# WHOIGit/ifcb_classifier

Measured on AMD Instinct MI355X. Metric: train images/sec, inception_v3 299^2 IFCB ROIs, higher is better.
Workload: dtype bf16; 1 GPU; inception_v3 100-class bf16 TRAIN, batch 256 per GPU, synthetic u8 ROIs h,w~U{32..299} resized on-GPU to 299x299 (BASELINE.json configs[1]); global_batch=256, parallelism=dp1, program_lanes=4, IFCBK_LANES=4, weight_gradient_lanes=1, optimizer=adam lr=1e-3, loss=CE + 0.4*CE_aux, input_pipeline=preprocess then step on one stream

## Files before the change

### ifcb_classifier_amd/csrc/conv_common.h

```cpp
#pragma once
#include "common.h"

namespace {

struct ConvArgs {
    const void* x;
    const void* w;
    void* y;
    float* part;
    const float* ep_scale;
    const float* ep_shift;
    const void* ep_res;
    int ep_ldr, ep_relu;
    const void* bs_raw;
    const float *bs_mean, *bs_invstd, *bs_scale, *bs_shift;
    int bs_ld;
    const void* pad_;
    unsigned xbytes, wbytes;
    int H, W, C, ldx;
    int K, R, S;
    int P, Q, ldy;
    int ostr_h, ostr_w, base_h, base_w, ish, isw;
    int M, Kg;
    int accumulate;
    int seg_n, seg_end[4], seg_ld[4], seg_aff[4];
    void* seg_y[4];
    int PQ;
    int tilesN;
    int wKg, wSfull, w_rbase, w_sbase;
    int oH, oW, o_a, o_b;
    fastdiv_t fPQ, fQ;
    int tr;
    fastdiv_t fP;
    int dbg;
};

typedef const __attribute__((address_space(1))) void* gptr_t;
typedef __attribute__((address_space(3))) void* lptr_t;

template <class T> struct Mma;
template <> struct Mma<bf16_t> {
    typedef bf16x8_t frag_t;
    __device__ static __forceinline__ void run(const frag_t& a, const frag_t& b, f32x4_t& c) {
        c = __builtin_amdgcn_mfma_f32_16x16x32_bf16(a, b, c, 0, 0, 0);
    }
    __device__ static __forceinline__ void pack4(bf16_t* p, const f32x4_t& v) {
        uint2 u;
        u.x = pack2bf(v[0], v[1]);
        u.y = pack2bf(v[2], v[3]);
        *reinterpret_cast<uint2*>(p) = u;
    }
};
template <> struct Mma<float> {
    typedef f32x4_t frag_t;
    __device__ static __forceinline__ void run(const frag_t& a, const frag_t& b, f32x4_t& c) {
#pragma unroll
        for (int j = 0; j < 4; ++j) c = __builtin_amdgcn_mfma_f32_16x16x4f32(a[j], b[j], c, 0, 0, 0);
    }
    __device__ static __forceinline__ void pack4(float* p, const f32x4_t& v) { *reinterpret_cast<f32x4_t*>(p) = v; }
};

__device__ __forceinline__ void lds_dma16(__amdgpu_buffer_rsrc_t rs, lptr_t dst, unsigned voff, int soff) {
    __builtin_amdgcn_raw_ptr_buffer_load_lds(rs, dst, 16, voff, soff, 0, 0);
}

template <int N>
__device__ __forceinline__ void wait_vmcnt() {
    asm volatile("s_waitcnt vmcnt(%0)" ::"n"(N) : "memory");
}


template <class T, int BM, int BN, int NTHREADS, int MODE>
__device__ __forceinline__ void conv_epilogue_store(const ConvArgs& a, T* sC, float* sRed, const int t, const int lane, const int wave,
                                                    const int m0, const int n0, const int mtile) {
    constexpr bool BSTAT = MODE == 3;
    constexpr int ES = (int)sizeof(T);
    constexpr int CE = 16 / ES;
    constexpr int NW = NTHREADS / 64;
    constexpr int CPR = BN / CE;
    constexpr int CPRP = CPR <= 4 ? 4 : CPR <= 8 ? 8 : CPR <= 16 ? 16 : 32;
    constexpr int LDC = BN + CE;
    {
        constexpr int RPP = NTHREADS / CPRP;
        const int cc = t & (CPRP - 1);
        const int r0 = t / CPRP;
        const bool cvalid = (cc < CPR) && (n0 + cc * CE < a.K);
        typedef float f32x2_t __attribute__((ext_vector_type(2)));
        f32x2_t s1p[CE / 2], s2p[CE / 2];
#pragma unroll
        for (int j = 0; j < CE / 2; ++j) s1p[j] = s2p[j] = f32x2_t{0.f, 0.f};
        if (cvalid) {
            const int nn = n0 + cc * CE;
            float bmu[CE], bis[CE], bsc[CE], bsh[CE];
            if (BSTAT) {
#pragma unroll
                for (int j = 0; j < CE; ++j) {
                    bmu[j] = a.bs_mean[nn + j];
                    bis[j] = a.bs_invstd[nn + j];
                    bsc[j] = a.bs_scale[nn + j];
                    bsh[j] = a.bs_shift[nn + j];
                }
            }
            float sc[CE], sh[CE];
            if (a.ep_scale) {
#pragma unroll
                for (int j = 0; j < CE; ++j) {
                    sc[j] = a.ep_scale[nn + j];
                    sh[j] = a.ep_shift[nn + j];
                }
            }
            T* segbase = (T*)a.y + nn;
            int segld = a.ldy;
            bool seg_aff = true;
            if (MODE == 4) {
                int si = 0;
#pragma unroll
                for (int q = 0; q < 3; ++q)
                    if (q + 1 < a.seg_n && nn >= a.seg_end[q]) si = q + 1;
                segbase = (T*)a.seg_y[si] + (nn - (si ? a.seg_end[si - 1] : 0));
// ... 128 lines not shown
```

### ifcb_classifier_amd/csrc/conv_igemm.hip

```cpp
#include "conv_common.h"
#include <stdlib.h>

namespace {

template <class T, int NT, int WM, int NSTAGE, int MODE>
__global__ __launch_bounds__(128 * WM) void conv_igemm(ConvArgs a) {
    constexpr bool STRIDED = MODE == 1;
    constexpr int ES = (int)sizeof(T);
    constexpr int CE = 16 / ES;
    constexpr int BK = 128 / ES;
    typedef typename Mma<T>::frag_t frag_t;
    constexpr int NW = 2 * WM;
    constexpr int NTHREADS = 64 * NW;
    constexpr int BM = 64 * WM;
    constexpr int BN = 32 * NT;
    constexpr int JB = (NT * 4 + NW - 1) / NW;
    constexpr int G = 4 + JB;
    constexpr int D = NSTAGE - 1;
    constexpr int LDC = BN + CE;
    constexpr int STAGE = (BM + BN) * BK;
    constexpr int STAGE_BYTES = NSTAGE * STAGE * ES;
    constexpr int CT_BYTES = BM * LDC * ES + NW * BN * 2 * 4;
    constexpr int MAIN_BYTES = STAGE_BYTES > CT_BYTES ? STAGE_BYTES : CT_BYTES;
    constexpr int DUMMY_BYTES = (JB * NW > NT * 4) ? 1024 : 0;
    __shared__ __attribute__((aligned(16))) unsigned char smem[MAIN_BYTES + DUMMY_BYTES];
    T* sStage = reinterpret_cast<T*>(smem);
    T* sC = reinterpret_cast<T*>(smem);
    float* sRed = reinterpret_cast<float*>(smem + BM * LDC * ES);
    T* sDummy = reinterpret_cast<T*>(smem + MAIN_BYTES);

    const int t = threadIdx.x;
    const int lane = t & 63;
    const int wave = __builtin_amdgcn_readfirstlane(t >> 6);
    const int wm = wave >> 1, wn = wave & 1;
    const int bid = (int)xcd_remap(blockIdx.x, gridDim.x);
    const int mtile = bid / a.tilesN, ntile = bid - mtile * a.tilesN;
    const int m0 = mtile * BM, n0 = ntile * BN;

    const __amdgpu_buffer_rsrc_t rsA = __builtin_amdgcn_make_buffer_rsrc((void*)a.x, 0, a.xbytes, 0x00020000);
    const __amdgpu_buffer_rsrc_t rsB = __builtin_amdgcn_make_buffer_rsrc((void*)a.w, 0, a.wbytes, 0x00020000);
    constexpr unsigned OOB = 0x80000000u;
    const int lrow8 = lane >> 3;
    const int csrc = (lane & 7) ^ lrow8;
    int off0[4], bh[4], bw[4];
#pragma unroll
    for (int j = 0; j < 4; ++j) {
        int m = m0 + (wave * 4 + j) * 8 + lrow8;
        bool rv = m < a.M;
        int mm = rv ? m : 0;
        int n = (int)fdiv((uint32_t)mm, a.fPQ);
        int rem = mm - n * a.PQ;
        int p = (int)fdiv((uint32_t)rem, a.fQ);
        int q = rem - p * a.Q;
        bh[j] = rv ? p * a.ostr_h + a.base_h : -(1 << 24);
        bw[j] = q * a.ostr_w + a.base_w;
        off0[j] = STRIDED ? n * a.H * a.W * a.ldx : ((n * a.H + bh[j]) * a.W + bw[j]) * a.ldx;
    }
    int kc, kr, ks, tapoff;
    {
        kc = csrc * CE;
        kr = 0;
        ks = 0;
        while (kc >= a.C) {
            kc -= a.C;
            if (++ks == a.S) { ks = 0; ++kr; }
        }
        tapoff = (kr * a.W + ks) * a.ldx + kc;
    }
    int wk = MODE == 2 ? ((a.w_rbase + 2 * kr) * a.wSfull + a.w_sbase + 2 * ks) * a.C + kc : 0;
    unsigned woff[JB];
    bool gvalid[JB];
#pragma unroll
    for (int j = 0; j < JB; ++j) {
        int grp = j * NW + wave;
        gvalid[j] = grp < NT * 4;
        int n = n0 + grp * 8 + lrow8;
        woff[j] = (gvalid[j] && n < a.K) ? (MODE == 2 ? (unsigned)(n * a.wKg) : (unsigned)(n * a.Kg + csrc * CE)) * (unsigned)ES : OOB;
    }
    const int nk = (a.Kg + BK - 1) / BK;
    const int hmask = (1 << a.ish) - 1, wmask = (1 << a.isw) - 1;
    const int rowstep = a.W * a.ldx, colwrap = a.S * a.ldx;
    const int wrowskip = MODE == 2 ? (2 * a.wSfull - 2 * a.S) * a.C : 0;

    const bool plain = (MODE == 0 || MODE == 3 || MODE == 4) && a.R == 1 && a.S == 1 && a.base_h == 0 && a.base_w == 0;
    unsigned va[4];
#pragma unroll
    for (int j = 0; j < 4; ++j) va[j] = bh[j] >= 0 ? (unsigned)(off0[j] + csrc * CE) * (unsigned)ES : OOB;
    const bool ktail_ok = (nk - 1) * BK + csrc * CE < a.Kg;

#define ISSUE_TILE(kt, stage)                                                                              \
    {                                                                                                      \
        T* dstA = sStage + (stage) * STAGE;                                                                \
        T* dstB = dstA + BM * BK;                                                                          \
        if (plain) {                                                                                       \
            const bool cut = (kt) == nk - 1 && !ktail_ok;                                                  \
            _Pragma("unroll") for (int j = 0; j < 4; ++j)                                                  \
                lds_dma16(rsA, (lptr_t)(dstA + (wave * 4 + j) * 8 * BK), cut ? OOB : va[j], (kt) * 128);   \
        } else {                                                                                           \
            const bool kvalid = kr < a.R;                                                                  \
            _Pragma("unroll") for (int j = 0; j < 4; ++j) {                                                \
                int hr = bh[j] + kr, wr = bw[j] + ks;                                                      \
                unsigned voff;                                                                             \
                if (STRIDED) {                                                                             \
                    bool v = kvalid && hr >= 0 && wr >= 0 && ((hr & hmask) == 0) && ((wr & wmask) == 0);   \
                    int hi = hr >> a.ish, wi = wr >> a.isw;                                                \
                    v = v && hi < a.H && wi < a.W;                                                         \
                    voff = v ? (unsigned)(off0[j] + (hi * a.W + wi) * a.ldx + kc) * (unsigned)ES : OOB;    \
                } else {                                                                                   \
                    bool v = kvalid && (unsigned)hr < (unsigned)a.H && (unsigned)wr < (unsigned)a.W;       \
                    voff = v ? (unsigned)(off0[j] + tapoff) * (unsigned)ES : OOB;                          \
                }                                                                                          \
                __builtin_amdgcn_raw_ptr_buffer_load_lds(rsA, (lptr_t)(dstA + (wave * 4 + j) * 8 * BK), 16, voff, 0, 0, 0); \
            }                                                                                              \
        }                                                                                                  \
        if (MODE == 2) {                                                                                   \
            const bool kv2 = ((kt) * BK + csrc * CE) < a.Kg;                                               \
            _Pragma("unroll") for (int j = 0; j < JB; ++j) {                                               \
                unsigned voff = (kv2 && woff[j] != OOB) ? woff[j] + (unsigned)wk * (unsigned)ES : OOB;     \
// ... 246 lines not shown
                    sh[j] = nv ? a.ep_shift[ncol + nt * 16 + j] : 0.f;
                }
            }
            f32x2_t s1[2] = {f32x2_t{0.f, 0.f}, f32x2_t{0.f, 0.f}}, s2[2] = {f32x2_t{0.f, 0.f}, f32x2_t{0.f, 0.f}};
#pragma unroll
            for (int mt = 0; mt < 4; ++mt) {
                f32x4_t v = acc[nt][mt];
                if (a.ep_scale) {
#pragma unroll
                    for (int j = 0; j < 4; ++j) {
                        v[j] = bf2f(f2bf(v[j])) * sc[j] + sh[j];
                        if (a.ep_relu) v[j] = fmaxf(v[j], 0.f);
                    }
                }
                uint2 u;
                u.x = pack2bf(v[0], v[1]);
                u.y = pack2bf(v[2], v[3]);
                if (mv[mt] && nv) *reinterpret_cast<uint2*>(row[mt] + nt * 16) = u;
                const f32x2_t lo = {__uint_as_float(u.x << 16), __uint_as_float(u.x & 0xffff0000u)};
                const f32x2_t hi = {__uint_as_float(u.y << 16), __uint_as_float(u.y & 0xffff0000u)};
                s1[0] += lo; s1[1] += hi;
                s2[0] += lo * lo; s2[1] += hi * hi;
            }
            if (a.part) {
#pragma unroll
                for (int off = 1; off < 16; off <<= 1)
#pragma unroll
                    for (int h = 0; h < 2; ++h)
#pragma unroll
                        for (int j = 0; j < 2; ++j) {
                            s1[h][j] += __shfl_xor(s1[h][j], off);
                            s2[h][j] += __shfl_xor(s2[h][j], off);
                        }
                if (frow == 0 && nv) {
                    float* prow = a.part + ((size_t)(mtile * 2 + wm) * 2) * a.K + ncol + nt * 16;
#pragma unroll
                    for (int j = 0; j < 4; ++j) {
                        prow[j] = s1[j >> 1][j & 1];
                        prow[a.K + j] = s2[j >> 1][j & 1];
                    }
                }
            }
        }
    }
}

int pick_nt(int K, int maxnt) {
    static int force = -1;
    if (force < 0) { const char* e = getenv("IFCBK_CONV_NT"); force = e ? atoi(e) : 0; }
    if (force > 0 && force <= maxnt) return force;
    int best = 1;
    long bestc = -1;
    for (int nt = 1; nt <= maxnt; ++nt) {
        int bn = 32 * nt;
        long c = (long)cdiv(K, bn) * (bn + 48);
        if (bestc < 0 || c < bestc || (c == bestc && nt > best)) { bestc = c; best = nt; }
    }
    return best;
}

int check_desc(ifcbk_ctx* ctx, const ifcbk_conv_desc* d, bool dgrad = false) {
    if (!d) IFCBK_FAIL(ctx, IFCBK_EINVAL, "conv: null desc");
    if (d->dtype != IFCBK_BF16 && d->dtype != IFCBK_F32) IFCBK_FAIL(ctx, IFCBK_EUNSUPPORTED, "conv: dtype must be bf16 or f32");
    const int ce = dtype_chunk(d->dtype), es = dtype_esize(d->dtype);
    if (d->C % ce || d->K % ce || d->ldx % ce || d->ldy % ce || d->C <= 0 || d->K <= 0)
        IFCBK_FAIL(ctx, IFCBK_EINVAL, "conv: C=%d K=%d ldx=%d ldy=%d must be positive multiples of %d", d->C, d->K, d->ldx, d->ldy, ce);
    if (d->stride_h < 1 || d->stride_w < 1 || (dgrad && (d->stride_h > 2 || d->stride_w > 2)))
        IFCBK_FAIL(ctx, IFCBK_EINVAL, "conv: stride must be >= 1 (1 or 2 for the input gradient)");
    int P = (d->H + 2 * d->pad_h - d->R) / d->stride_h + 1, Q = (d->W + 2 * d->pad_w - d->S) / d->stride_w + 1;
    if (P != d->P || Q != d->Q) IFCBK_FAIL(ctx, IFCBK_EINVAL, "conv: P,Q=%d,%d inconsistent (expect %d,%d)", d->P, d->Q, P, Q);
    if ((int64_t)d->N * d->P * d->Q * d->ldy * es >= (1ll << 31) || (int64_t)d->N * d->H * d->W * d->ldx * es >= (1ll << 31))
        IFCBK_FAIL(ctx, IFCBK_EINVAL, "conv: a tensor exceeds the 2 GiB buffer-descriptor window");
    return 0;
}

int pick_wm(int M, int K) {
    static int force = -1;
    if (force < 0) { const char* e = getenv("IFCBK_CONV_WM"); force = e ? atoi(e) : 0; }
    (void)M; (void)K;
    return force == 4 ? 4 : 2;
}

template <class T, int NT, int WM, int NSTAGE>
void launch(const ConvArgs& a, hipStream_t st) {
    int tilesM = cdiv(a.M, 64 * WM);
    dim3 grid((unsigned)(tilesM * a.tilesN)), block(128 * WM);
    if (a.seg_n) hipLaunchKernelGGL((conv_igemm<T, NT, WM, NSTAGE, 4>), grid, block, 0, st, a);
    else if (a.bs_raw) hipLaunchKernelGGL((conv_igemm<T, NT, WM, NSTAGE, 3>), grid, block, 0, st, a);
    else if (a.wKg) hipLaunchKernelGGL((conv_igemm<T, NT, WM, NSTAGE, 2>), grid, block, 0, st, a);
    else if (a.ish | a.isw) hipLaunchKernelGGL((conv_igemm<T, NT, WM, NSTAGE, 1>), grid, block, 0, st, a);
    else hipLaunchKernelGGL((conv_igemm<T, NT, WM, NSTAGE, 0>), grid, block, 0, st, a);
}

int ws_min_steps() {
    static int v = -1;
    if (v < 0) { const char* e = getenv("IFCBK_CONV_WS"); v = e ? atoi(e) : 4; }
    return v;
}
int num_cus();
int ws_max_tiles() {
    static int v = -1;
    if (v < 0) { const char* e = getenv("IFCBK_CONV_WS_TILES"); v = e ? atoi(e) : 2 * num_cus(); }
    return v;
}
bool ws_shape_ok(int dtype, int M, int K, int Kg) {
    const int ms = ws_min_steps();
    if (ms <= 0 || dtype != IFCBK_BF16 || pick_wm(M, K) != 2 || cdiv(Kg, 64) < ms) return false;
    const int nt = pick_nt(K, 6);
    return (int64_t)cdiv(M, 128) * cdiv(K, 32 * nt) <= ws_max_tiles();
}
int num_cus() {
    static int n = 0;
    if (!n) {
        int dev = 0;
        hipDeviceProp_t pr;
        if (hipGetDevice(&dev) == hipSuccess && hipGetDeviceProperties(&pr, dev) == hipSuccess) n = pr.multiProcessorCount;
        if (n <= 0) n = 256;
    }
    return n;
}

template <int NT>
void launch_ws(const ConvArgs& a, hipStream_t st) {
    const int total = cdiv(a.M, 128) * a.tilesN;
    const int grid = total < num_cus() ? total : num_cus();
    hipLaunchKernelGGL((conv_ws<NT>), dim3((unsigned)grid), dim3(512), 0, st, a, total);
}

bool big_ok(const ConvArgs& a) { return !a.wKg && !(a.ish | a.isw); }
bool pp3_ok(const ConvArgs& a) {
    return big_ok(a) && !a.seg_n && !a.bs_raw && !a.accumulate && !a.ep_res && (a.ep_scale == nullptr || a.part == nullptr);
}

int run(ifcbk_ctx* ctx, ConvArgs& a, int dtype, hipStream_t st) {
    const bool f32 = dtype == IFCBK_F32;
    if (!a.wKg && !(a.ish | a.isw) && a.ostr_h == 1 && a.ostr_w == 1 && !a.seg_n && !a.accumulate && !a.ep_res && a.PQ > 0) {
        const int N = a.M / a.PQ;
        if (ifcbk_conv_flat_rows(dtype, N, a.H, a.W, a.C, a.K, a.R, a.S, -a.base_h, -a.base_w, a.P, a.Q) > 0)
            return ifcbk_conv_flat_launch(ctx, &a, N, st);
    }
    if (big_ok(a) && a.ostr_h == 1 && a.ostr_w == 1 && !a.seg_n && a.PQ > 0) {
        const int N = a.M / a.PQ;
        if (ifcbk_conv_slab_plan(dtype, N, a.H, a.W, a.C, a.K, a.R, a.S, -a.base_h, -a.base_w, a.P, a.Q) > 0)
            return ifcbk_conv_slab_launch(ctx, &a, N, st);
    }
    if (pp3_ok(a) && ifcbk_conv_pp3_plan(dtype, a.M, a.K, a.Kg, a.ep_scale ? 1 : 0)) return ifcbk_conv_pp3_launch(ctx, &a, st);
    {
        int bmt = 0, btn = 0;
        if (big_ok(a) && ifcbk_conv_big_plan(dtype, a.M, a.K, a.Kg, &bmt, &btn)) return ifcbk_conv_big_launch(ctx, &a, bmt, btn, st);
    }
    int wm = f32 ? 2 : pick_wm(a.M, a.K);
    int nt = pick_nt(a.K, f32 ? 4 : (wm == 4 ? 5 : 6));
    a.tilesN = cdiv(a.K, 32 * nt);
    if ((int64_t)cdiv(a.M, 64 * wm) * a.tilesN >= (1ll << 31)) IFCBK_FAIL(ctx, IFCBK_EINVAL, "conv: grid too large");
    if (ws_shape_ok(dtype, a.M, a.K, a.Kg) && !a.seg_n && !a.bs_raw && !a.wKg && !(a.ish | a.isw) && !a.accumulate && !a.ep_res) {
        switch (nt) {
            case 1: launch_ws<1>(a, st); break;
            case 2: launch_ws<2>(a, st); break;
            case 3: launch_ws<3>(a, st); break;
            case 4: launch_ws<4>(a, st); break;
            case 5: launch_ws<5>(a, st); break;
            default: launch_ws<6>(a, st); break;
        }
        IFCBK_LAUNCH_CHECK(ctx, "conv_ws");
        return 0;
    }
    if (f32) {
        switch (nt) {
            case 1: launch<float, 1, 2, 2>(a, st); break;
            case 2: launch<float, 2, 2, 2>(a, st); break;
            case 3: launch<float, 3, 2, 2>(a, st); break;
            default: launch<float, 4, 2, 2>(a, st); break;
        }
    } else if (wm == 4) {
        switch (nt) {
            case 1: launch<bf16_t, 1, 4, 3>(a, st); break;
            case 2: launch<bf16_t, 2, 4, 3>(a, st); break;
            case 3: launch<bf16_t, 3, 4, 3>(a, st); break;
            case 4: launch<bf16_t, 4, 4, 3>(a, st); break;
            default: launch<bf16_t, 5, 4, 3>(a, st); break;
        }
    } else {
        switch (nt) {
            case 1: launch<bf16_t, 1, 2, 2>(a, st); break;
            case 2: launch<bf16_t, 2, 2, 2>(a, st); break;
            case 3: launch<bf16_t, 3, 2, 2>(a, st); break;
            case 4: launch<bf16_t, 4, 2, 2>(a, st); break;
            case 5: launch<bf16_t, 5, 2, 2>(a, st); break;
            default: launch<bf16_t, 6, 2, 2>(a, st); break;
        }
    }
    IFCBK_LAUNCH_CHECK(ctx, "conv_igemm");
    return 0;
}

}

int ifcbk_num_cus() { return num_cus(); }

int ifcbk_conv_fwd_nt(int K, int M) { return pick_nt(K, pick_wm(M, K) == 4 ? 5 : 6); }

int ifcbk_conv_f32_nt(int K) { return pick_nt(K, 4); }

int ifcbk_conv_fwd_wm(int M, int K) { return pick_wm(M, K); }

bool ifcbk_conv_ws_shape(int dtype, int M, int K, int Kg) { return ws_shape_ok(dtype, M, K, Kg); }

static bool fwd_rows(const ifcbk_conv_desc* d) {
    return ifcbk_conv_rows_ok(d->dtype, d->C, d->K, d->R, d->S, d->stride_h, d->stride_w, d->pad_h, d->pad_w, d->Q);
}

extern "C" int ifcbk_conv2d_fwd_mblocks(const ifcbk_conv_desc* d) {
    if (fwd_rows(d)) return ifcbk_conv_rows_blocks(d->N, d->P);
    int M = d->N * d->P * d->Q;
    if (d->stride_h == 1 && d->stride_w == 1)
        if (int fs = ifcbk_conv_flat_rows(d->dtype, d->N, d->H, d->W, d->C, d->K, d->R, d->S, d->pad_h, d->pad_w, d->P, d->Q)) return fs;
    if (d->stride_h == 1 && d->stride_w == 1)
        if (int smt = ifcbk_conv_slab_plan(d->dtype, d->N, d->H, d->W, d->C, d->K, d->R, d->S, d->pad_h, d->pad_w, d->P, d->Q)) return cdiv(M, 32 * smt);
    if (ifcbk_conv_pp3_plan(d->dtype, M, d->K, d->R * d->S * d->C, 0)) return 2 * cdiv(M, 256);
    {
        int bmt = 0, btn = 0;
        if (ifcbk_conv_big_plan(d->dtype, M, d->K, d->R * d->S * d->C, &bmt, &btn)) return cdiv(M, 32 * bmt);
    }
    if (ws_shape_ok(d->dtype, M, d->K, d->R * d->S * d->C)) return 2 * cdiv(M, 128);
    return cdiv(M, 64 * pick_wm(M, d->K));
}

struct FwdSegs { int n, end[4], ld[4], aff[4]; void* y[4]; };
static int conv_fwd_impl(ifcbk_ctx* ctx, const ifcbk_conv_desc* d, const void* x, const void* w, void* y, float* bn_part,
                         const float* scale, const float* shift, const void* residual, int ldr, int relu, void* stream,
                         const FwdSegs* seg = nullptr);

extern "C" int ifcbk_conv2d_fwd_affine_segments(ifcbk_ctx* ctx, const ifcbk_conv_desc* d, const void* x, const void* w, int nseg,
                                                void* const* ys, const int32_t* ldys, const int32_t* ksegs, const int32_t* affine,
                                                const float* scale, const float* shift, void* stream) {
    if (!d || nseg < 1 || nseg > 4 || !ys || !ldys || !ksegs || !affine || !scale || !shift)
        IFCBK_FAIL(ctx, IFCBK_EINVAL, "conv2d_fwd_affine_segments: bad args");
    FwdSegs sg;
    sg.n = nseg;
    int end = 0;
    const int ce = dtype_chunk(d->dtype);
    for (int q = 0; q < 4; ++q) {
        const bool live = q < nseg;
        if (live) {
            if (!ys[q] || ksegs[q] <= 0 || ksegs[q] % ce || ldys[q] % ce)
                IFCBK_FAIL(ctx, IFCBK_EINVAL, "conv2d_fwd_affine_segments: segment %d: null / size not a multiple of %d", q, ce);
            end += ksegs[q];
        }
        sg.end[q] = end; sg.ld[q] = live ? ldys[q] : 0; sg.aff[q] = live ? affine[q] : 0; sg.y[q] = live ? ys[q] : nullptr;
    }
    if (end != d->K) IFCBK_FAIL(ctx, IFCBK_EINVAL, "conv2d_fwd_affine_segments: segment sizes sum to %d, K=%d", end, d->K);
    return conv_fwd_impl(ctx, d, x, w, ys[0], nullptr, scale, shift, nullptr, 0, 1, stream, &sg);
}

extern "C" int ifcbk_conv2d_fwd(ifcbk_ctx* ctx, const ifcbk_conv_desc* d, const void* x, const void* w, void* y,
                                float* bn_part, void* stream) {
    return conv_fwd_impl(ctx, d, x, w, y, bn_part, nullptr, nullptr, nullptr, 0, 0, stream);
}

extern "C" int ifcbk_conv2d_fwd_affine(ifcbk_ctx* ctx, const ifcbk_conv_desc* d, const void* x, const void* w, void* y,
                                       const float* scale, const float* shift, const void* residual, int ldr, int relu,
                                       void* stream) {
    if (!scale || !shift) IFCBK_FAIL(ctx, IFCBK_EINVAL, "conv2d_fwd_affine: scale/shift required");
    return conv_fwd_impl(ctx, d, x, w, y, nullptr, scale, shift, residual, ldr, relu, stream);
}

extern "C" int ifcbk_conv2d_fwd_affine_maxpool_ok(const ifcbk_conv_desc* d) {
    return d && ifcbk_conv_rows_pool_ok(d->dtype, d->C, d->K, d->R, d->S, d->stride_h, d->stride_w, d->pad_h, d->pad_w, d->P, d->Q) ? 1 : 0;
}

extern "C" int ifcbk_conv2d_fwd_affine_maxpool(ifcbk_ctx* ctx, const ifcbk_conv_desc* d, const void* x, const void* w, void* y_pooled,
                                               int ldp, const float* scale, const float* shift, int relu, void* stream) {
    if (!ifcbk_conv2d_fwd_affine_maxpool_ok(d)) IFCBK_FAIL(ctx, IFCBK_EUNSUPPORTED, "conv2d_fwd_affine_maxpool: not served by the row-streaming kernel");
    if (!x || !w || !y_pooled || !scale || !shift || ldp < d->K || ldp % 8) IFCBK_FAIL(ctx, IFCBK_EINVAL, "conv2d_fwd_affine_maxpool: bad operand");
    {
        ifcbk_conv_desc one = *d;
// ... 54 lines not shown
    a.seg_n = seg ? seg->n : 0;
    for (int q = 0; q < 4; ++q) {
        a.seg_end[q] = seg ? seg->end[q] : 0; a.seg_ld[q] = seg ? seg->ld[q] : 0; a.seg_aff[q] = seg ? seg->aff[q] : 0;
        a.seg_y[q] = seg ? seg->y[q] : nullptr;
    }
    const int es = dtype_esize(d->dtype);
    a.xbytes = (unsigned)((int64_t)d->N * d->H * d->W * d->ldx * es); a.wbytes = (unsigned)((int64_t)d->K * d->R * d->S * d->C * es);
    a.H = d->H; a.W = d->W; a.C = d->C; a.ldx = d->ldx;
    a.K = d->K; a.R = d->R; a.S = d->S;
    a.P = d->P; a.Q = d->Q; a.ldy = d->ldy;
    a.ostr_h = d->stride_h; a.ostr_w = d->stride_w; a.base_h = -d->pad_h; a.base_w = -d->pad_w;
    a.ish = 0; a.isw = 0;
    a.wKg = 0; a.wSfull = 0; a.w_rbase = 0; a.w_sbase = 0; a.oH = 0; a.oW = 0; a.o_a = 0; a.o_b = 0;
    a.M = d->N * d->P * d->Q; a.Kg = d->R * d->S * d->C; a.accumulate = 0; a.PQ = d->P * d->Q;
    a.fPQ = make_fastdiv(a.PQ); a.fQ = make_fastdiv(a.Q);
    return run(ctx, a, d->dtype, (hipStream_t)stream);
}

struct BnStatArgs {
    const void* raw;
    int ld;
    const float *mean, *invstd, *scale, *shift;
    float* part;
};

static bool dgrad_bnstat_ok(const ifcbk_conv_desc* d) {
    if (d->stride_h != 1 || d->stride_w != 1) return false;
    return !ifcbk_conv_rows_ok(d->dtype, d->K, d->C, d->R, d->S, d->stride_h, d->stride_w, 2 - d->pad_h, 2 - d->pad_w, d->W);
}

static int dgrad_impl(ifcbk_ctx* ctx, const ifcbk_conv_desc* d, const void* dy, const void* wT, void* dx, int accumulate,
                      const BnStatArgs* bs, void* stream);

extern "C" int ifcbk_conv2d_dgrad(ifcbk_ctx* ctx, const ifcbk_conv_desc* d, const void* dy, const void* wT, void* dx,
                                  int accumulate, void* stream) {
    return dgrad_impl(ctx, d, dy, wT, dx, accumulate, nullptr, stream);
}

extern "C" int ifcbk_conv2d_dgrad_bnstat_mblocks(const ifcbk_conv_desc* d) {
    if (!d || !dgrad_bnstat_ok(d)) return 0;
    int M = d->N * d->H * d->W;
    if (int fs = ifcbk_conv_flat_rows(d->dtype, d->N, d->P, d->Q, d->K, d->C, d->R, d->S, d->R - 1 - d->pad_h, d->S - 1 - d->pad_w, d->H, d->W)) return fs;
    if (int smt = ifcbk_conv_slab_plan(d->dtype, d->N, d->P, d->Q, d->K, d->C, d->R, d->S, d->R - 1 - d->pad_h, d->S - 1 - d->pad_w, d->H, d->W)) return cdiv(M, 32 * smt);
    {
        int bmt = 0, btn = 0;
        if (ifcbk_conv_big_plan(d->dtype, M, d->C, d->R * d->S * d->K, &bmt, &btn)) return cdiv(M, 32 * bmt);
    }
    return cdiv(M, 64 * pick_wm(M, d->C));
}

extern "C" int ifcbk_conv2d_dgrad_bnstat(ifcbk_ctx* ctx, const ifcbk_conv_desc* d, const void* dy, const void* wT, void* dx,
                                         const void* prev_raw, int prev_ld, const float* prev_mean, const float* prev_invstd,
                                         const float* prev_scale, const float* prev_shift, float* part, void* stream) {
    if (!d || !dgrad_bnstat_ok(d)) IFCBK_FAIL(ctx, IFCBK_EUNSUPPORTED, "conv2d_dgrad_bnstat: stride-1 implicit-GEMM input gradients only");
    if (!prev_raw || !prev_mean || !prev_invstd || !prev_scale || !prev_shift || !part)
        IFCBK_FAIL(ctx, IFCBK_EINVAL, "conv2d_dgrad_bnstat: null operand");
    BnStatArgs bs = {prev_raw, prev_ld, prev_mean, prev_invstd, prev_scale, prev_shift, part};
    return dgrad_impl(ctx, d, dy, wT, dx, 0, &bs, stream);
}

static int dgrad_impl(ifcbk_ctx* ctx, const ifcbk_conv_desc* d, const void* dy, const void* wT, void* dx, int accumulate,
                      const BnStatArgs* bs, void* stream) {
    if (int e = check_desc(ctx, d, true)) return e;
    if (!bs && !accumulate && ifcbk_conv_rows_ok(d->dtype, d->K, d->C, d->R, d->S, d->stride_h, d->stride_w, 2 - d->pad_h, 2 - d->pad_w, d->W))
        return ifcbk_conv_rows_launch(ctx, d->K, d->C, d->N, d->P, d->Q, d->ldy, d->H, d->W, d->ldx, 2 - d->pad_h, 2 - d->pad_w, dy,
                                      wT, dx, nullptr, nullptr, nullptr, 0, (hipStream_t)stream);
    ConvArgs a;
    a.dbg = 0; a.tr = 0; a.fP = make_fastdiv(1);
    a.ep_scale = nullptr; a.ep_shift = nullptr; a.ep_res = nullptr; a.ep_ldr = 0; a.ep_relu = 0;
    a.x = dy; a.w = wT; a.y = dx; a.part = bs ? bs->part : nullptr;
    a.seg_n = 0;
    a.bs_raw = bs ? bs->raw : nullptr; a.bs_ld = bs ? bs->ld : 0;
    a.bs_mean = bs ? bs->mean : nullptr; a.bs_invstd = bs ? bs->invstd : nullptr;
    a.bs_scale = bs ? bs->scale : nullptr; a.bs_shift = bs ? bs->shift : nullptr;
    const int es = dtype_esize(d->dtype);
    a.xbytes = (unsigned)((int64_t)d->N * d->P * d->Q * d->ldy * es); a.wbytes = (unsigned)((int64_t)d->K * d->R * d->S * d->C * es);
    a.H = d->P; a.W = d->Q; a.C = d->K; a.ldx = d->ldy;
    a.K = d->C; a.R = d->R; a.S = d->S;
    a.P = d->H; a.Q = d->W; a.ldy = d->ldx;
    a.ostr_h = 1; a.ostr_w = 1;
    a.wKg = 0; a.wSfull = 0; a.w_rbase = 0; a.w_sbase = 0; a.oH = 0; a.oW = 0; a.o_a = 0; a.o_b = 0;
    a.accumulate = accumulate;
    if (d->stride_h == 2 && d->stride_w == 2 && d->R >= 2 && d->S >= 2 && d->H >= 2 && d->W >= 2) {
        for (int pa = 0; pa < 2; ++pa)
            for (int pb = 0; pb < 2; ++pb) {
                const int r0 = (pa + d->pad_h) & 1, s0 = (pb + d->pad_w) & 1;
                const int nU = (d->R - r0 + 1) / 2, nV = (d->S - s0 + 1) / 2;
                const int Hc = (d->H - pa + 1) / 2, Wc = (d->W - pb + 1) / 2;
                ConvArgs c = a;
                c.R = nU; c.S = nV;
                c.P = Hc; c.Q = Wc;
                c.base_h = (pa + d->pad_h - r0) / 2 - (nU - 1);
                c.base_w = (pb + d->pad_w - s0) / 2 - (nV - 1);
                c.ish = 0; c.isw = 0;
                c.wKg = d->R * d->S * d->K; c.wSfull = d->S;
                c.w_rbase = d->R - 1 - r0 - 2 * (nU - 1); c.w_sbase = d->S - 1 - s0 - 2 * (nV - 1);
                c.oH = d->H; c.oW = d->W; c.o_a = pa; c.o_b = pb;
                c.M = d->N * Hc * Wc; c.Kg = nU * nV * d->K; c.PQ = Hc * Wc;
                c.fPQ = make_fastdiv(c.PQ); c.fQ = make_fastdiv(c.Q);
                if (int e = run(ctx, c, d->dtype, (hipStream_t)stream)) return e;
            }
        return 0;
    }
    a.base_h = -(d->R - 1 - d->pad_h); a.base_w = -(d->S - 1 - d->pad_w);
    a.ish = d->stride_h == 2 ? 1 : 0; a.isw = d->stride_w == 2 ? 1 : 0;
    a.M = d->N * d->H * d->W; a.Kg = d->R * d->S * d->K; a.PQ = d->H * d->W;
    a.fPQ = make_fastdiv(a.PQ); a.fQ = make_fastdiv(a.Q);
    return run(ctx, a, d->dtype, (hipStream_t)stream);
}
```

### ifcb_classifier_amd/engine.py

```python
import ctypes as C
import math
import os

import torch

from . import _lib
from ._lib import Op, ConvDesc, BnDesc, PoolDesc, HeadDesc, RoiDesc


_DISPATCH_SWITCHES = ('IFCBK_CONV_PP3', 'IFCBK_CONV_PP3_GRID', 'IFCBK_WGRAD_LANE', 'IFCBK_WGRAD_GROUP', 'IFCBK_WGRAD_GROUP_MINKH', 'IFCBK_CONV_BIG', 'IFCBK_CONV_SLAB', 'IFCBK_CONV_BIG_MT', 'IFCBK_CONV_BIG_TN', 'IFCBK_CONV_FLAT', 'IFCBK_CONV_NT',
                      'IFCBK_CONV_WM', 'IFCBK_CONV_WS', 'IFCBK_CONV_WS_TILES', 'IFCBK_CONV_ROWS', 'IFCBK_WGRAD_PP',
                      'IFCBK_WGRAD_PP_KH', 'IFCBK_WGRAD_COLS', 'IFCBK_WGRAD_STEM', 'IFCBK_WGRAD_ROUNDS', 'IFCBK_WGRAD_FLAT',
                      'IFCBK_BN_BWD_ROWS')


def _dispatch_env():
    return tuple(os.environ.get(k) for k in _DISPATCH_SWITCHES)


def dtype_is_bf16(eng):
    return eng.dtype == 'bf16'


def _vp(t, byte_off=0):
    return None if t is None else C.c_void_p(t.data_ptr() + byte_off)


class OpList:

    def __init__(self):
        self.ops = []
        self.tags = []
        self.meta = []

    def add(self, kind, tag, p=(), i=(), f=(), flags=0, conv=None, bn=None, pool=None, head=None, lane=0, reads=None,
            writes=None):
        o = Op()
        o.kind, o.flags = kind, flags
        self.meta.append((lane, reads, writes))
        for k, v in enumerate(p):
            o.p[k] = v if (v is None or isinstance(v, int)) else v.value
        for k, v in enumerate(i):
            o.i[k] = int(v)
        for k, v in enumerate(f):
            o.f[k] = float(v)
        if conv is not None:
            o.u.conv = conv
        elif bn is not None:
            o.u.bn = bn
        elif pool is not None:
            o.u.pool = pool
        elif head is not None:
            o.u.head = head
        self.ops.append(o)
        self.tags.append(tag)
        return o

    def extend(self, other):
        self.ops.extend(other.ops)
        self.tags.extend(other.tags)
        self.meta.extend(other.meta)

    def slice(self, b0, b1):
        sub = OpList()
        sub.ops, sub.tags, sub.meta = self.ops[b0:b1], self.tags[b0:b1], self.meta[b0:b1]
        return sub

    def freeze(self):
        arr = (Op * len(self.ops))(*self.ops)
        for k, (lane, wait) in enumerate(schedule_lanes(self.meta)):
            arr[k].flags = (arr[k].flags & 0xff) | (lane << 8) | (wait << 12)
        return arr


def _overlap(a, b):
    return a[:-2] == b[:-2] and a[-2] < b[-1] and b[-2] < a[-1]


def schedule_lanes(meta):
    NL = 8
    count = [0] * NL
    synced = [[0] * NL for _ in range(NL)]
    table = {}
    star = ('*', 0, 1)
    out = []
    for lane, reads, writes in meta:
        if reads is None and writes is None:
            lane, reads, writes = 0, [star], [star]
        else:
            reads, writes = list(reads or ()) + [star], list(writes or ())
        deps = set()
        for r in reads:
            for res, (w, _rd) in table.items():
                if w is not None and _overlap(r, res):
                    deps.add(w)
        for wres in writes:
# ... 1541 lines not shown
```

Baseline: 12210 images/s.

## Fuse four stride-2 dgrad parity-class launches into one grid

For stride-2 input-gradient convolutions, the four parity sub-convolutions used to be launched one after another as separate igemm kernels. They now go out as a single launch whose blocks are split across the classes, ordered by Kg descending so the longest tiles start first. Each block looks up its class parameters from a small per-class table. This is meant to cut launch overhead and the tail-idle gaps between the small per-class grids, at the cost of a larger kernel argument and some per-block class lookup. It is on by default but only applies when all four classes pick the same tile config, and it skips the flat/big/ws paths the per-class run() might have chosen.

After: 12250 images/s (median of 6 runs). No clear change (+0.3%).

```diff
diff --git a/ifcb_classifier_amd/csrc/conv_common.h b/ifcb_classifier_amd/csrc/conv_common.h
--- a/ifcb_classifier_amd/csrc/conv_common.h
+++ b/ifcb_classifier_amd/csrc/conv_common.h
@@ -35,6 +35,18 @@
     int dbg;
 };
 
+struct S2Class {
+    int R, S, P, Q, base_h, base_w, w_rbase, w_sbase, o_a, o_b, M, Kg, PQ, first;
+    fastdiv_t fPQ, fQ;
+};
+struct ConvArgsS2 {
+    ConvArgs a;
+    int n;
+    S2Class cls[4];
+};
+template <int MODE> struct IgemmArgs { typedef ConvArgs type; };
+template <> struct IgemmArgs<2> { typedef ConvArgsS2 type; };
+
 typedef const __attribute__((address_space(1))) void* gptr_t;
 typedef __attribute__((address_space(3))) void* lptr_t;
 
diff --git a/ifcb_classifier_amd/csrc/conv_igemm.hip b/ifcb_classifier_amd/csrc/conv_igemm.hip
--- a/ifcb_classifier_amd/csrc/conv_igemm.hip
+++ b/ifcb_classifier_amd/csrc/conv_igemm.hip
@@ -1,10 +1,37 @@
 #include "conv_common.h"
 #include <stdlib.h>
+#include <string.h>
 
 namespace {
 
+__device__ __forceinline__ const ConvArgs& block_args(const ConvArgs& ka, int& bid) {
+    bid = (int)xcd_remap(blockIdx.x, gridDim.x);
+    return ka;
+}
+__device__ __forceinline__ ConvArgs block_args(const ConvArgsS2& ka, int& bid) {
+    ConvArgs a = ka.a;
+    if (ka.n == 0) {
+        bid = (int)xcd_remap(blockIdx.x, gridDim.x);
+        return a;
+    }
+    const int b = (int)blockIdx.x;
+    int c = 0;
+#pragma unroll
+    for (int q = 1; q < 4; ++q)
+        if (q < ka.n && b >= ka.cls[q].first) c = q;
+    const S2Class& k = ka.cls[c];
+    const int end = c + 1 < ka.n ? ka.cls[c + 1].first : (int)gridDim.x;
+    bid = (int)xcd_remap((unsigned)(b - k.first), (unsigned)(end - k.first));
+    a.R = k.R; a.S = k.S; a.P = k.P; a.Q = k.Q; a.base_h = k.base_h; a.base_w = k.base_w;
+    a.w_rbase = k.w_rbase; a.w_sbase = k.w_sbase; a.o_a = k.o_a; a.o_b = k.o_b;
+    a.M = k.M; a.Kg = k.Kg; a.PQ = k.PQ; a.fPQ = k.fPQ; a.fQ = k.fQ;
+    return a;
+}
+
 template <class T, int NT, int WM, int NSTAGE, int MODE>
-__global__ __launch_bounds__(128 * WM) void conv_igemm(ConvArgs a) {
+__global__ __launch_bounds__(128 * WM) void conv_igemm(const typename IgemmArgs<MODE>::type ka) {
+    int bid;
+    const ConvArgs& a = block_args(ka, bid);
     constexpr bool STRIDED = MODE == 1;
     constexpr int ES = (int)sizeof(T);
     constexpr int CE = 16 / ES;
@@ -33,7 +60,6 @@
     const int lane = t & 63;
     const int wave = __builtin_amdgcn_readfirstlane(t >> 6);
     const int wm = wave >> 1, wn = wave & 1;
-    const int bid = (int)xcd_remap(blockIdx.x, gridDim.x);
     const int mtile = bid / a.tilesN, ntile = bid - mtile * a.tilesN;
     const int m0 = mtile * BM, n0 = ntile * BN;
 
@@ -446,13 +472,21 @@
 }
 
 template <class T, int NT, int WM, int NSTAGE>
-void launch(const ConvArgs& a, hipStream_t st) {
+void launch(const ConvArgs& a, hipStream_t st, const ConvArgsS2* s2 = nullptr) {
     int tilesM = cdiv(a.M, 64 * WM);
     dim3 grid((unsigned)(tilesM * a.tilesN)), block(128 * WM);
-    if (a.seg_n) hipLaunchKernelGGL((conv_igemm<T, NT, WM, NSTAGE, 4>), grid, block, 0, st, a);
+    if (s2) {
+        const S2Class& l = s2->cls[s2->n - 1];
+        grid.x = (unsigned)(l.first + cdiv(l.M, 64 * WM) * a.tilesN);
+        hipLaunchKernelGGL((conv_igemm<T, NT, WM, NSTAGE, 2>), grid, block, 0, st, *s2);
+    } else if (a.seg_n) hipLaunchKernelGGL((conv_igemm<T, NT, WM, NSTAGE, 4>), grid, block, 0, st, a);
     else if (a.bs_raw) hipLaunchKernelGGL((conv_igemm<T, NT, WM, NSTAGE, 3>), grid, block, 0, st, a);
-    else if (a.wKg) hipLaunchKernelGGL((conv_igemm<T, NT, WM, NSTAGE, 2>), grid, block, 0, st, a);
-    else if (a.ish | a.isw) hipLaunchKernelGGL((conv_igemm<T, NT, WM, NSTAGE, 1>), grid, block, 0, st, a);
+    else if (a.wKg) {
+        ConvArgsS2 one;
+        one.a = a; one.n = 0;
+        memset(one.cls, 0, sizeof(one.cls));
+        hipLaunchKernelGGL((conv_igemm<T, NT, WM, NSTAGE, 2>), grid, block, 0, st, one);
+    } else if (a.ish | a.isw) hipLaunchKernelGGL((conv_igemm<T, NT, WM, NSTAGE, 1>), grid, block, 0, st, a);
     else hipLaunchKernelGGL((conv_igemm<T, NT, WM, NSTAGE, 0>), grid, block, 0, st, a);
 }
 
@@ -496,8 +530,41 @@
     return big_ok(a) && !a.seg_n && !a.bs_raw && !a.accumulate && !a.ep_res && (a.ep_scale == nullptr || a.part == nullptr);
 }
 
+void igemm_tile(const ConvArgs& a, int dtype, int* wm, int* nt) {
+    const bool f32 = dtype == IFCBK_F32;
+    *wm = f32 ? 2 : pick_wm(a.M, a.K);
+    *nt = pick_nt(a.K, f32 ? 4 : (*wm == 4 ? 5 : 6));
+}
+
+void launch_igemm(const ConvArgs& a, int dtype, int wm, int nt, hipStream_t st, const ConvArgsS2* s2) {
+    if (dtype == IFCBK_F32) {
+        switch (nt) {
+            case 1: launch<float, 1, 2, 2>(a, st, s2); break;
+            case 2: launch<float, 2, 2, 2>(a, st, s2); break;
+            case 3: launch<float, 3, 2, 2>(a, st, s2); break;
+            default: launch<float, 4, 2, 2>(a, st, s2); break;
+        }
+    } else if (wm == 4) {
+        switch (nt) {
+            case 1: launch<bf16_t, 1, 4, 3>(a, st, s2); break;
+            case 2: launch<bf16_t, 2, 4, 3>(a, st, s2); break;
+            case 3: launch<bf16_t, 3, 4, 3>(a, st, s2); break;
+            case 4: launch<bf16_t, 4, 4, 3>(a, st, s2); break;
+            default: launch<bf16_t, 5, 4, 3>(a, st, s2); break;
+        }
+    } else {
+        switch (nt) {
+            case 1: launch<bf16_t, 1, 2, 2>(a, st, s2); break;
+            case 2: launch<bf16_t, 2, 2, 2>(a, st, s2); break;
+            case 3: launch<bf16_t, 3, 2, 2>(a, st, s2); break;
+            case 4: launch<bf16_t, 4, 2, 2>(a, st, s2); break;
+            case 5: launch<bf16_t, 5, 2, 2>(a, st, s2); break;
+            default: launch<bf16_t, 6, 2, 2>(a, st, s2); break;
+        }
+    }
+}
+
 int run(ifcbk_ctx* ctx, ConvArgs& a, int dtype, hipStream_t st) {
-    const bool f32 = dtype == IFCBK_F32;
     if (!a.wKg && !(a.ish | a.isw) && a.ostr_h == 1 && a.ostr_w == 1 && !a.seg_n && !a.accumulate && !a.ep_res && a.PQ > 0) {
         const int N = a.M / a.PQ;
         if (ifcbk_conv_flat_rows(dtype, N, a.H, a.W, a.C, a.K, a.R, a.S, -a.base_h, -a.base_w, a.P, a.Q) > 0)
@@ -513,8 +580,8 @@
         int bmt = 0, btn = 0;
         if (big_ok(a) && ifcbk_conv_big_plan(dtype, a.M, a.K, a.Kg, &bmt, &btn)) return ifcbk_conv_big_launch(ctx, &a, bmt, btn, st);
     }
-    int wm = f32 ? 2 : pick_wm(a.M, a.K);
-    int nt = pick_nt(a.K, f32 ? 4 : (wm == 4 ? 5 : 6));
+    int wm, nt;
+    igemm_tile(a, dtype, &wm, &nt);
     a.tilesN = cdiv(a.K, 32 * nt);
     if ((int64_t)cdiv(a.M, 64 * wm) * a.tilesN >= (1ll << 31)) IFCBK_FAIL(ctx, IFCBK_EINVAL, "conv: grid too large");
     if (ws_shape_ok(dtype, a.M, a.K, a.Kg) && !a.seg_n && !a.bs_raw && !a.wKg && !(a.ish | a.isw) && !a.accumulate && !a.ep_res) {
@@ -529,33 +596,45 @@
         IFCBK_LAUNCH_CHECK(ctx, "conv_ws");
         return 0;
     }
-    if (f32) {
-        switch (nt) {
-            case 1: launch<float, 1, 2, 2>(a, st); break;
-            case 2: launch<float, 2, 2, 2>(a, st); break;
-            case 3: launch<float, 3, 2, 2>(a, st); break;
-            default: launch<float, 4, 2, 2>(a, st); break;
-        }
-    } else if (wm == 4) {
-        switch (nt) {
-            case 1: launch<bf16_t, 1, 4, 3>(a, st); break;
-            case 2: launch<bf16_t, 2, 4, 3>(a, st); break;
-            case 3: launch<bf16_t, 3, 4, 3>(a, st); break;
-            case 4: launch<bf16_t, 4, 4, 3>(a, st); break;
-            default: launch<bf16_t, 5, 4, 3>(a, st); break;
-        }
-    } else {
-        switch (nt) {
-            case 1: launch<bf16_t, 1, 2, 2>(a, st); break;
-            case 2: launch<bf16_t, 2, 2, 2>(a, st); break;
-            case 3: launch<bf16_t, 3, 2, 2>(a, st); break;
-            case 4: launch<bf16_t, 4, 2, 2>(a, st); break;
-            case 5: launch<bf16_t, 5, 2, 2>(a, st); break;
-            default: launch<bf16_t, 6, 2, 2>(a, st); break;
-        }
-    }
+    launch_igemm(a, dtype, wm, nt, st, nullptr);
     IFCBK_LAUNCH_CHECK(ctx, "conv_igemm");
     return 0;
+}
+
+bool s2_grid_on() {
+    const char* e = getenv("IFCBK_DGRAD_S2_GRID");
+    return !e || atoi(e) != 0;
+}
+
+int run_s2_grid(ifcbk_ctx* ctx, const ConvArgs* c, int dtype, hipStream_t st) {
+    if (!s2_grid_on()) return 0;
+    int wm, nt;
+    igemm_tile(c[0], dtype, &wm, &nt);
+    int order[4] = {0, 1, 2, 3};
+    for (int i = 1; i < 4; ++i) {
+        int w2, n2;
+        igemm_tile(c[i], dtype, &w2, &n2);
+        if (w2 != wm || n2 != nt) return 0;
+        for (int j = i; j > 0 && c[order[j]].Kg > c[order[j - 1]].Kg; --j) { int t = order[j]; order[j] = order[j - 1]; order[j - 1] = t; }
+    }
+    ConvArgsS2 s;
+    s.a = c[order[0]];
+    s.a.tilesN = cdiv(s.a.K, 32 * nt);
+    s.n = 4;
+    int64_t first = 0;
+    for (int i = 0; i < 4; ++i) {
+        const ConvArgs& k = c[order[i]];
+        S2Class& q = s.cls[i];
+        q.R = k.R; q.S = k.S; q.P = k.P; q.Q = k.Q; q.base_h = k.base_h; q.base_w = k.base_w;
+        q.w_rbase = k.w_rbase; q.w_sbase = k.w_sbase; q.o_a = k.o_a; q.o_b = k.o_b;
+        q.M = k.M; q.Kg = k.Kg; q.PQ = k.PQ; q.fPQ = k.fPQ; q.fQ = k.fQ;
+        q.first = (int)first;
+        first += (int64_t)cdiv(k.M, 64 * wm) * s.a.tilesN;
+        if (first >= (1ll << 31)) return 0;
+    }
+    launch_igemm(s.a, dtype, wm, nt, st, &s);
+    IFCBK_LAUNCH_CHECK(ctx, "conv_igemm (stride-2 classes)");
+    return 1;
 }
 
 }
@@ -776,12 +855,14 @@
     a.wKg = 0; a.wSfull = 0; a.w_rbase = 0; a.w_sbase = 0; a.oH = 0; a.oW = 0; a.o_a = 0; a.o_b = 0;
     a.accumulate = accumulate;
     if (d->stride_h == 2 && d->stride_w == 2 && d->R >= 2 && d->S >= 2 && d->H >= 2 && d->W >= 2) {
+        ConvArgs cls[4];
         for (int pa = 0; pa < 2; ++pa)
             for (int pb = 0; pb < 2; ++pb) {
                 const int r0 = (pa + d->pad_h) & 1, s0 = (pb + d->pad_w) & 1;
                 const int nU = (d->R - r0 + 1) / 2, nV = (d->S - s0 + 1) / 2;
                 const int Hc = (d->H - pa + 1) / 2, Wc = (d->W - pb + 1) / 2;
-                ConvArgs c = a;
+                ConvArgs& c = cls[pa * 2 + pb];
+                c = a;
                 c.R = nU; c.S = nV;
                 c.P = Hc; c.Q = Wc;
                 c.base_h = (pa + d->pad_h - r0) / 2 - (nU - 1);
@@ -792,8 +873,10 @@
                 c.oH = d->H; c.oW = d->W; c.o_a = pa; c.o_b = pb;
                 c.M = d->N * Hc * Wc; c.Kg = nU * nV * d->K; c.PQ = Hc * Wc;
                 c.fPQ = make_fastdiv(c.PQ); c.fQ = make_fastdiv(c.Q);
-                if (int e = run(ctx, c, d->dtype, (hipStream_t)stream)) return e;
             }
+        if (const int g = run_s2_grid(ctx, cls, d->dtype, (hipStream_t)stream)) return g < 0 ? g : 0;
+        for (int i = 0; i < 4; ++i)
+            if (int e = run(ctx, cls[i], d->dtype, (hipStream_t)stream)) return e;
         return 0;
     }
     a.base_h = -(d->R - 1 - d->pad_h); a.base_w = -(d->S - 1 - d->pad_w);
diff --git a/ifcb_classifier_amd/engine.py b/ifcb_classifier_amd/engine.py
--- a/ifcb_classifier_amd/engine.py
+++ b/ifcb_classifier_amd/engine.py
@@ -11,7 +11,7 @@
 _DISPATCH_SWITCHES = ('IFCBK_CONV_PP3', 'IFCBK_CONV_PP3_GRID', 'IFCBK_WGRAD_LANE', 'IFCBK_WGRAD_GROUP', 'IFCBK_WGRAD_GROUP_MINKH', 'IFCBK_CONV_BIG', 'IFCBK_CONV_SLAB', 'IFCBK_CONV_BIG_MT', 'IFCBK_CONV_BIG_TN', 'IFCBK_CONV_FLAT', 'IFCBK_CONV_NT',
                       'IFCBK_CONV_WM', 'IFCBK_CONV_WS', 'IFCBK_CONV_WS_TILES', 'IFCBK_CONV_ROWS', 'IFCBK_WGRAD_PP',
                       'IFCBK_WGRAD_PP_KH', 'IFCBK_WGRAD_COLS', 'IFCBK_WGRAD_STEM', 'IFCBK_WGRAD_ROUNDS', 'IFCBK_WGRAD_FLAT',
-                      'IFCBK_BN_BWD_ROWS')
+                      'IFCBK_BN_BWD_ROWS', 'IFCBK_DGRAD_S2_GRID')
 
 
 def _dispatch_env():
```
